# treangenlab/Seqwin

Measured on AMD Instinct MI355X. Metric: Gbp/s minimizer-indexed, higher is better.
Workload: dtype u64

## Files before the change

seqwin_amd/csrc/radix.hip:

```cpp
#include <algorithm>
#include <cstdlib>
#include <cstring>
#include <vector>
#include <map>
#include <mutex>

#include "device.hpp"

namespace sw {
namespace {

constexpr int RS_ITEMS = 16;
#ifdef SW_RS_STAMPS
__device__ unsigned long long *g_rs_stamps = nullptr;
#define RS_STAMP(i)                                                                                        \
    do {                                                                                                   \
        if (g_rs_stamps && (tile & 63u) == 0 && threadIdx.x == 0) g_rs_stamps[(size_t)(tile >> 6) * 16 + (i)] = clock64(); \
    } while (0)
#else
#define RS_STAMP(i) do { } while (0)
#endif
#ifndef RS_LOOK
#define RS_LOOK 4
#endif
// ... 954 lines not shown
        if (!slot) slot = new StateBuf;
        b = slot;
    }
    StateUse u(*b, std::unique_lock<std::mutex>(b->mu));
    if (b->words < words) {
        if (b->p) (void)hipFree(b->p);
        b->p = nullptr;
        b->words = 0;
        const size_t want = words + words / 4;
        SW_HIP(hipMalloc(&b->p, want * 8));
        b->words = want;
        b->epoch = 0;
        SW_HIP(hipMemsetAsync(b->p, 0, want * 8, stream));
    }
    return u;
}
uint32_t next_epoch(StateBuf &b, hipStream_t stream)
{
    if (++b.epoch >= 0xFFFFu) {
        SW_HIP(hipMemsetAsync(b.p, 0, b.words * 8, stream));
        b.epoch = 1;
    }
    return b.epoch;
}

template <int THREADS, int BITS>
void sort_passes(uint64_t *&keys, uint64_t *&alt, uint64_t n, unsigned begin_bit, unsigned end_bit, hipStream_t stream, uint32_t *d_fail,
                 bool perm_hi32, unsigned long long *d_hist_given)
{
    constexpr uint32_t RADIX = 1u << BITS, TILE = THREADS * RS_ITEMS;
    const unsigned n_passes = (end_bit - begin_bit + BITS - 1) / BITS;
    const uint64_t n_tiles = (n + TILE - 1) / TILE;
    const char *kind = SW_AB_GETENV("SEQWIN_AMD_RADIX_KERNEL");
    const bool persistent = !(kind && !strcmp(kind, "classic"));
    uint32_t dbg = 0;
#ifdef SW_RADIX_ABLATION
    if (const char *e = getenv("SEQWIN_AMD_RADIX_DEBUG")) dbg = (uint32_t)atoi(e) & 15u;
#endif
    if (fault_rank()) dbg |= 16u;
    int grid_p = 0;
    if (persistent) {
        static std::mutex &mu = *new std::mutex;
        static std::map<int, int> &grids = *new std::map<int, int>;
        int dev = 0;
        SW_HIP(hipGetDevice(&dev));
        std::lock_guard<std::mutex> lock(mu);
        int &g = grids[dev];
        if (!g) {
            int per_cu = 0;
            hipDeviceProp_t prop;
            SW_HIP(hipGetDeviceProperties(&prop, dev));
            SW_HIP(hipOccupancyMaxActiveBlocksPerMultiprocessor(&per_cu, k_rs_pass_p<THREADS, BITS, 0>, THREADS, 0));
            g = std::max(1, per_cu) * std::max(1, prop.multiProcessorCount);
        }
        grid_p = g;
    }
    const bool atomic_rank = persistent && rank_mode() == 1;
    DevArray<unsigned long long> hist_own(d_hist_given ? 0 : (size_t)n_passes * RADIX), state(persistent ? 0 : (size_t)n_tiles * RADIX);
    std::unique_ptr<StateUse> su(persistent ? new StateUse(state_buf(stream, (size_t)n_tiles * RADIX)) : nullptr);
    StateBuf *sb = su ? &su->b : nullptr;
    struct { unsigned long long *p; } hist{d_hist_given ? d_hist_given : hist_own.p};
    const bool unstable = perm_hi32 && persistent && !SW_AB_GETENV("SEQWIN_AMD_RADIX_STABLE_UNSORT");
    DevArray<unsigned long long> cursor(unstable ? (size_t)RADIX * RS_CURSOR_STRIDE : 0);
    DevArray<uint32_t> tickets(n_passes);
    SW_HIP(hipMemsetAsync(tickets.p, 0, tickets.bytes(), stream));
    if (d_hist_given) {
    } else if (perm_hi32 && begin_bit >= 32) {
        hipLaunchKernelGGL(k_rs_perm_hist<BITS>, dim3(n_passes), dim3(RADIX), 0, stream, n, begin_bit, end_bit, hist.p);
    } else {
        SW_HIP(hipMemsetAsync(hist.p, 0, hist_own.bytes(), stream));
        hipLaunchKernelGGL(k_rs_hist<BITS>, dim3((unsigned)((n + 32767) / 32768)), dim3(256), 0, stream, keys, n, begin_bit, end_bit,
                           n_passes, hist.p);
    }
    SW_HIP(hipGetLastError());
#ifdef SW_RS_STAMPS
    DevArray<unsigned long long> stamps;
    const size_t n_st = (size_t)(n_tiles / 64 + 1) * 16;
    if (getenv("SEQWIN_AMD_STAMPS") && persistent) stamps.alloc(n_st);
#endif
    for (unsigned p = 0; p < n_passes; ++p) {
        const unsigned sh = begin_bit + BITS * p, bits = std::min<unsigned>(BITS, end_bit - sh);
#ifdef SW_RS_STAMPS
        if (stamps.p) {
            SW_HIP(hipMemsetAsync(stamps.p, 0, stamps.bytes(), stream));
            unsigned long long *ptr = stamps.p;
            SW_HIP(hipMemcpyToSymbolAsync(HIP_SYMBOL(g_rs_stamps), &ptr, sizeof ptr, 0, hipMemcpyHostToDevice, stream));
        }
#endif
        unsigned long long *cur = unstable && p == 0 ? cursor.p : nullptr;
        hipLaunchKernelGGL(k_rs_scan<BITS>, dim3(1), dim3(RADIX), 0, stream, hist.p + (size_t)p * RADIX, cur);
        if (!cur && !persistent) SW_HIP(hipMemsetAsync(state.p, 0, state.bytes(), stream));
        if (persistent) {
            const uint32_t epoch = cur ? 0u : next_epoch(*sb, stream);
            auto launch = [&](auto kern) {
                hipLaunchKernelGGL(kern, dim3((unsigned)std::min<uint64_t>(n_tiles, (uint64_t)grid_p)), dim3(THREADS), 0, stream, keys, alt, n,
                                   (uint32_t)n_tiles, sh, bits, hist.p + (size_t)p * RADIX, sb->p, tickets.p + p, d_fail, dbg, cur,
                                   RS_CURSOR_STRIDE, 64u, epoch);
            };
            if (cur ? !ballot_forced() : atomic_rank) launch(k_rs_pass_p<THREADS, BITS, 1>);
            else launch(k_rs_pass_p<THREADS, BITS, 0>);
        } else {
#ifdef SW_AB
            hipLaunchKernelGGL((k_rs_pass<THREADS, BITS>), dim3((unsigned)n_tiles), dim3(THREADS), 0, stream, keys, alt, n, sh, bits,
                               hist.p + (size_t)p * RADIX, state.p, d_fail);
#endif
        }
        SW_HIP(hipGetLastError());
#ifdef SW_RS_STAMPS
        if (stamps.p) {
            std::vector<unsigned long long> hs(n_st);
            SW_HIP(hipStreamSynchronize(stream));
            SW_HIP(hipMemcpy(hs.data(), stamps.p, stamps.bytes(), hipMemcpyDeviceToHost));
            double acc[8] = {0}, look[3] = {0};
            size_t cnt = 0;
            for (size_t t = 0; t + 16 <= n_st; t += 16) {
                if (!hs[t] || !hs[t + 7]) continue;
                for (int i = 1; i <= 7; ++i) acc[i] += (double)(hs[t + i] - hs[t + i - 1]);
                for (int i = 0; i < 3; ++i) look[i] += (double)hs[t + 8 + i];
                ++cnt;
            }
            static const char *nm[] = {"", "rank", "barrier", "totals+scan", "barrier+scatter", "lookback(d0)", "barrier", "write-out"};
            fprintf(stderr, "[rs stamps] %d x %d bits, pass %u, %zu tiles sampled; mean clocks:", THREADS, BITS, p, cnt);
            double sum = 0;
            for (int i = 1; i <= 7; ++i) { fprintf(stderr, " %s=%.0f", nm[i], cnt ? acc[i] / cnt : 0.0); sum += cnt ? acc[i] / cnt : 0.0; }
            fprintf(stderr, " | tile %.0f | look-back of digit 0: %.1f steps, %.1f polls of an unpublished record, %.1f records behind\n", sum,
                    cnt ? look[0] / cnt : 0.0, cnt ? look[1] / cnt : 0.0, cnt ? look[2] / cnt : 0.0);
        }
#endif
        std::swap(keys, alt);
    }
}

}

namespace {
__global__ void k_rs_perm_cursors(unsigned long long *__restrict__ cursor, uint32_t n_groups, uint32_t radix, uint32_t stride,
                                  unsigned group_bits, unsigned digit_shift)
{
    const uint32_t i = blockIdx.x * blockDim.x + threadIdx.x;
    if (i >= n_groups * radix) return;
    const uint64_t g = i / radix, d = i % radix;
    cursor[(size_t)i * stride] = (group_bits < 64 ? g << group_bits : 0ull) + (d << digit_shift);
}
}

bool radix_unsort_perm(uint64_t *&keys, uint64_t *&alt, uint64_t n, unsigned low_bits, unsigned nbit, hipStream_t stream, uint32_t *d_fail)
{
    constexpr int THREADS = 512, BITS = 8;
    constexpr uint32_t RADIX = 1u << BITS, TILE = THREADS * RS_ITEMS;
    if (n == 0 || nbit <= low_bits + 8 || nbit > low_bits + 16 || SW_AB_GETENV("SEQWIN_AMD_RADIX_STABLE_UNSORT")) return false;
    if ((1ull << (low_bits + 8)) % TILE) return false;
    const char *kind = SW_AB_GETENV("SEQWIN_AMD_RADIX_KERNEL");
    if (kind && !strcmp(kind, "classic")) return false;
    const unsigned hi_bits = nbit - low_bits - 8;
    const uint32_t n_groups = (uint32_t)((n + (1ull << (low_bits + 8)) - 1) >> (low_bits + 8));
    const uint64_t n_tiles = (n + TILE - 1) / TILE;
    int dev = 0, per_cu = 0;
    SW_HIP(hipGetDevice(&dev));
    hipDeviceProp_t prop;
    SW_HIP(hipGetDeviceProperties(&prop, dev));
    SW_HIP(hipOccupancyMaxActiveBlocksPerMultiprocessor(&per_cu, k_rs_pass_p<THREADS, BITS, 0>, THREADS, 0));
    const unsigned grid = (unsigned)std::min<uint64_t>(n_tiles, (uint64_t)std::max(1, per_cu) * std::max(1, prop.multiProcessorCount));
    DevArray<unsigned long long> cur_a((size_t)RADIX * RS_CURSOR_STRIDE), cur_b((size_t)n_groups * RADIX);
    DevArray<uint32_t> tickets(2);
    SW_HIP(hipMemsetAsync(tickets.p, 0, 8, stream));
    hipLaunchKernelGGL(k_rs_perm_cursors, dim3(1), dim3(RADIX), 0, stream, cur_a.p, 1u, RADIX, RS_CURSOR_STRIDE, 64u, low_bits + 8);
    hipLaunchKernelGGL(k_rs_perm_cursors, dim3((n_groups * RADIX + 255) / 256), dim3(256), 0, stream, cur_b.p, n_groups, RADIX, 1u,
                       low_bits + 8, low_bits);
    auto pass = ballot_forced() ? k_rs_pass_p<THREADS, BITS, 0> : k_rs_pass_p<THREADS, BITS, 1>;
    hipLaunchKernelGGL(pass, dim3(grid), dim3(THREADS), 0, stream, (const uint64_t *)keys, alt, n, (uint32_t)n_tiles,
                       32u + low_bits + 8, hi_bits, (const unsigned long long *)nullptr, (unsigned long long *)nullptr, tickets.p, d_fail,
                       0u, cur_a.p, RS_CURSOR_STRIDE, 64u, 0u);
    std::swap(keys, alt);
    hipLaunchKernelGGL(pass, dim3(grid), dim3(THREADS), 0, stream, (const uint64_t *)keys, alt, n, (uint32_t)n_tiles, 32u + low_bits,
                       8u, (const unsigned long long *)nullptr, (unsigned long long *)nullptr, tickets.p + 1, d_fail, 0u, cur_b.p, 1u,
                       low_bits + 8, 0u);
    std::swap(keys, alt);
    SW_HIP(hipGetLastError());
    return true;
}

bool radix_pairs_available() { return rank_mode() == 1; }
int radix_rank_mode() { return rank_mode(); }

uint64_t radix_trim_state()
{
    uint64_t freed = 0;
    if (g_state_uses) return 0;
    std::lock_guard<std::mutex> lock(state_registry_mu());
    for (auto &kv : state_registry()) {
        StateBuf &b = *kv.second;
        std::unique_lock<std::mutex> use(b.mu, std::try_to_lock);
        if (!use.owns_lock() || !b.p) continue;
        int cur = -1;
        (void)hipGetDevice(&cur);
        if (cur != kv.first.first) (void)hipSetDevice(kv.first.first);
        (void)hipFree(b.p);
        if (cur != kv.first.first && cur >= 0) (void)hipSetDevice(cur);
        freed += b.words * 8;
        b.p = nullptr;
        b.words = 0;
        b.epoch = 0;
    }
    return freed;
}

void radix_demote_rank()
{
    int dev = 0;
    SW_HIP(hipGetDevice(&dev));
    std::lock_guard<std::mutex> lock(rank_mu());
    rank_modes()[dev] = 0;
}

void radix_sort_pairs32(uint32_t *&keys, uint32_t *&keys_alt, OccPay *&vals, OccPay *&vals_alt, uint64_t n, unsigned end_bit,
                        hipStream_t stream, uint32_t *d_fail, const StageSource *src, const std::function<void()> &after_first,
                        uint32_t *low_out)
{
    constexpr uint32_t RADIX = 1u << RP_BITS, TILE = RP_THREADS * RP_ITEMS;
    if (n == 0 || end_bit == 0) return;
    if (end_bit > 32 || end_bit % RP_BITS) raise(SW_ERR_RUNTIME, "radix_sort_pairs32: key bits must be a multiple of 8 up to 32");
    if (n >= 0xFFFFFFFFull) raise(SW_ERR_RUNTIME, "radix_sort_pairs32: more than 2^32-2 elements");
    const unsigned n_passes = end_bit / RP_BITS;
    const uint64_t n_tiles = (n + TILE - 1) / TILE;
    int grid_p = 0;
    {
        static std::mutex &mu = *new std::mutex;
        static std::map<int, int> &grids = *new std::map<int, int>;
        int dev = 0;
        SW_HIP(hipGetDevice(&dev));
        std::lock_guard<std::mutex> lock(mu);
        int &g = grids[dev];
        if (!g) {
            int per_cu = 0;
            hipDeviceProp_t prop;
            SW_HIP(hipGetDeviceProperties(&prop, dev));
            SW_HIP(hipOccupancyMaxActiveBlocksPerMultiprocessor(&per_cu, k_rs_pair_pass<0>, RP_THREADS, 0));
            g = std::max(1, per_cu) * std::max(1, prop.multiProcessorCount);
        }
        grid_p = g;
    }
    DevArray<unsigned long long> hist((size_t)n_passes * RADIX);
    DevArray<uint32_t> tickets(n_passes);
    SW_HIP(hipMemsetAsync(tickets.p, 0, tickets.bytes(), stream));
    SW_HIP(hipMemsetAsync(hist.p, 0, hist.bytes(), stream));
    StageSource stage{};
    DevArray<uint32_t> chunk_tile;
    DevArray<unsigned long long> chunk_dir;
    if (src && src->rows) {
        stage = *src;
        hipLaunchKernelGGL(k_rs_hist32_rows, dim3((unsigned)((n + 16383) / 16384)), dim3(256), 0, stream,
                           reinterpret_cast<const uint4 *>(src->rows), n, n_passes, hist.p);
    } else if (src) {
        constexpr uint64_t CHUNK = 64 * RP_ITEMS;
        static_assert(TILE == (RP_THREADS / 64) * CHUNK, "a tile is one chunk per wave");
        const uint64_t n_chunks = (n + CHUNK - 1) / CHUNK;
        stage = *src;
        chunk_tile.alloc(n_chunks);
        chunk_dir.alloc(n_chunks * STAGE_ROW);
        stage.chunk_dir = chunk_dir.p;
        hipLaunchKernelGGL(k_rs_chunk_tiles, dim3((stage.n_tiles + 255u) / 256u), dim3(256), 0, stream, stage.tile_count, stage.dst_off,
                           stage.n_tiles, chunk_tile.p);
        hipLaunchKernelGGL(k_rs_stage_prepare, dim3((unsigned)std::min<uint64_t>(2048, (n_chunks + 3) / 4)), dim3(256), 0, stream, stage,
                           (const uint32_t *)chunk_tile.p, n, n_passes, chunk_dir.p, hist.p);
    } else {
        hipLaunchKernelGGL(k_rs_hist32, dim3((unsigned)((n + 65535) / 65536)), dim3(256), 0, stream, keys, n, n_passes, hist.p);
    }
    SW_HIP(hipGetLastError());
    StateUse su = state_buf(stream, (size_t)n_tiles * RADIX);
    StateBuf &sb = su.b;
    const StageSource none{};
    const uint32_t fault = fault_rank();
    for (unsigned p = 0; p < n_passes; ++p) {
        hipLaunchKernelGGL(k_rs_scan<RP_BITS>, dim3(1), dim3(RADIX), 0, stream, hist.p + (size_t)p * RADIX, (unsigned long long *)nullptr);
        const uint32_t epoch = next_epoch(sb, stream);
        const dim3 grid((unsigned)std::min<uint64_t>(n_tiles, (uint64_t)grid_p));
        if (p == 0 && src) {
            auto first = src->rows ? k_rs_pair_pass<2> : k_rs_pair_pass<1>;
            hipLaunchKernelGGL(first, grid, dim3(RP_THREADS), 0, stream, (const uint32_t *)nullptr, (const uint4 *)nullptr,
                               keys_alt, reinterpret_cast<uint4 *>(vals_alt), n, (uint32_t)n_tiles, 0u,
                               (const unsigned long long *)hist.p, sb.p, epoch, tickets.p, d_fail, stage,
                               n_passes == 1 ? low_out : (uint32_t *)nullptr, fault);
            SW_HIP(hipGetLastError());
            if (after_first) after_first();
        } else {
            hipLaunchKernelGGL(k_rs_pair_pass<0>, grid, dim3(RP_THREADS), 0, stream, (const uint32_t *)keys,
                               reinterpret_cast<const uint4 *>(vals), keys_alt, reinterpret_cast<uint4 *>(vals_alt), n, (uint32_t)n_tiles,
                               RP_BITS * p, (const unsigned long long *)(hist.p + (size_t)p * RADIX), sb.p, epoch, tickets.p + p, d_fail,
                               none, p + 1 == n_passes ? low_out : (uint32_t *)nullptr, fault);
            SW_HIP(hipGetLastError());
        }
        std::swap(keys, keys_alt);
        std::swap(vals, vals_alt);
    }
}

namespace {
constexpr uint32_t EB_RADIX = 512, EB_TABLE = EB_RADIX * EB_RADIX, EB_THREADS = 512;
constexpr uint64_t EB_EMPTY = ~0ull;
static_assert(EB_THREADS == EB_RADIX, "k_eb_finish: one bin per thread");
enum : uint32_t { EB_F_OVERFLOW = 1u, EB_F_RANGE = 2u, EB_F_ORDER = 4u };
struct EbInfo {
    unsigned long long n_sentinels;
    uint32_t n_tiles2, max_bucket, flags, n_runs;
};

__global__ __launch_bounds__(EB_RADIX) void k_eb_level1(const unsigned long long *__restrict__ h1, uint32_t tile_keys,
                                                        unsigned long long *__restrict__ cursor, unsigned long long *__restrict__ segtab,
                                                        EbInfo *__restrict__ info)
{
    __shared__ unsigned long long s[EB_RADIX];
    __shared__ uint32_t st[EB_RADIX];
    const uint32_t d = threadIdx.x;
    const unsigned long long c = h1[d];
    const uint32_t tiles = (uint32_t)((c + tile_keys - 1) / tile_keys);
    s[d] = c;
    st[d] = tiles;
    __syncthreads();
    for (uint32_t o = 1; o < EB_RADIX; o <<= 1) {
        const unsigned long long a = d >= o ? s[d - o] : 0;
        const uint32_t b = d >= o ? st[d - o] : 0;
        __syncthreads();
        s[d] += a;
        st[d] += b;
        __syncthreads();
    }
    const unsigned long long first = s[d] - c;
    cursor[(size_t)d * RS_CURSOR_STRIDE] = first;
    uint32_t w = st[d] - tiles;
    for (uint32_t t = 0; t < tiles; ++t)
        segtab[w + t] = seg_pack(first + (uint64_t)t * tile_keys, d, (uint32_t)min((unsigned long long)tile_keys, c - (uint64_t)t * tile_keys));
    if (d == EB_RADIX - 1) info->n_tiles2 = st[d];
}

__global__ __launch_bounds__(1024) void k_eb_count(const uint64_t *__restrict__ in, const unsigned long long *__restrict__ segtab,
                                                   const EbInfo *__restrict__ info, unsigned shift, uint32_t dmask, uint64_t sentinel,
                                                   uint32_t *__restrict__ table, EbInfo *__restrict__ out)
{
    __shared__ uint32_t hist[EB_RADIX];
    __shared__ uint32_t s_sent;
    const uint32_t n_tiles = info->n_tiles2;
    for (uint32_t w = blockIdx.x; w < n_tiles; w += gridDim.x) {
        const unsigned long long seg = segtab[w];
        const uint64_t first = seg_first(seg);
        const uint32_t cnt = seg_count(seg);
        if (threadIdx.x < EB_RADIX) hist[threadIdx.x] = 0;
        if (threadIdx.x == 0) s_sent = 0;
        __syncthreads();
        uint64_t key[RS_ITEMS];
#pragma unroll
        for (int i = 0; i < RS_ITEMS; ++i) {
            const uint32_t li = i * 1024 + threadIdx.x;
            key[i] = li < cnt ? in[first + li] : EB_EMPTY;
        }
        uint32_t sent = 0;
#pragma unroll
        for (int i = 0; i < RS_ITEMS; ++i) {
            if (key[i] == EB_EMPTY) continue;
            if (key[i] == sentinel) ++sent;
            atomicAdd(&hist[(uint32_t)(key[i] >> shift) & dmask], 1u);
        }
        if (sent) atomicAdd(&s_sent, sent);
        __syncthreads();
        if (threadIdx.x < EB_RADIX && hist[threadIdx.x]) atomicAdd(&table[seg_bucket(seg) * EB_RADIX + threadIdx.x], hist[threadIdx.x]);
        if (threadIdx.x == 0 && s_sent) atomicAdd(&out->n_sentinels, (unsigned long long)s_sent);
        __syncthreads();
    }
}

__global__ __launch_bounds__(1024) void k_eb_scan(const uint32_t *__restrict__ cnt, const unsigned long long *__restrict__ n_sent,
                                                  uint32_t sent_at, uint32_t *__restrict__ start, unsigned long long *__restrict__ cursor,
                                                  uint32_t *__restrict__ max_out, uint32_t *__restrict__ total_out)
{
    constexpr uint32_t PER4 = EB_TABLE / 1024 / 4;
    __shared__ uint32_t ws[16], wm[16];
    const uint32_t tid = threadIdx.x, lane = tid & 63u, wave = tid >> 6;
    const uint32_t sent = n_sent ? (uint32_t)*n_sent : 0u;
    const uint4 *cnt4 = reinterpret_cast<const uint4 *>(cnt) + (size_t)tid * PER4;
    uint32_t sum = 0, mx = 0;
#pragma unroll 16
    for (uint32_t j = 0; j < PER4; ++j) {
        const uint4 c = cnt4[j];
        mx = max(max(max(mx, c.x), max(c.y, c.z)), c.w);
        sum += c.x + c.y + c.z + c.w;
    }
    if (n_sent && sent_at / (4 * PER4) == tid) {
        mx = 0;
        for (uint32_t j = 0; j < 4 * PER4; ++j) {
            const uint32_t i = tid * 4 * PER4 + j, c = cnt[i];
            mx = max(mx, c - (i == sent_at ? min(c, sent) : 0u));
        }
    }
    uint32_t incl = sum;
    for (uint32_t o = 1; o < 64; o <<= 1) {
        const uint32_t up = __shfl_up(incl, o, 64);
        if (lane >= o) incl += up;
        mx = max(mx, __shfl_xor(mx, o, 64));
    }
    if (lane == 63) ws[wave] = incl;
    if (lane == 0) wm[wave] = mx;
    __syncthreads();
    uint32_t run = incl - sum;
    for (uint32_t w = 0; w < wave; ++w) run += ws[w];
    uint4 *start4 = reinterpret_cast<uint4 *>(start) + (size_t)tid * PER4;
    ulonglong2 *cur2 = reinterpret_cast<ulonglong2 *>(cursor) + (size_t)tid * PER4 * 2;
#pragma unroll 16
    for (uint32_t j = 0; j < PER4; ++j) {
        const uint4 c = cnt4[j];
        const uint4 st = make_uint4(run, run + c.x, run + c.x + c.y, run + c.x + c.y + c.z);
        start4[j] = st;
        if (cursor) {
            cur2[2 * j] = make_ulonglong2(st.x, st.y);
            cur2[2 * j + 1] = make_ulonglong2(st.z, st.w);
        }
        run = st.w + c.w;
    }
    if (tid == 1023) {
        start[EB_TABLE] = run;
        if (total_out) *total_out = run;
        uint32_t m = 0;
        for (uint32_t w = 0; w < 16; ++w) m = max(m, wm[w]);
        if (max_out) *max_out = m;
    }
}

__global__ __launch_bounds__(EB_THREADS) void k_eb_finish(const uint64_t *__restrict__ in, const uint32_t *__restrict__ start, uint32_t slots,
                                                          unsigned shift1, unsigned shift2, uint32_t mask2, unsigned bin_shift,
                                                          uint32_t bin_mask, uint64_t sentinel,
                                                          uint64_t *__restrict__ tk, uint32_t *__restrict__ tc,
                                                          uint32_t *__restrict__ n_distinct, uint32_t *__restrict__ flags)
{
    extern __shared__ __align__(16) unsigned char eb_lds[];
    unsigned long long *hk = reinterpret_cast<unsigned long long *>(eb_lds);
    uint32_t *hc = reinterpret_cast<uint32_t *>(hk + slots);
    uint16_t *idx = reinterpret_cast<uint16_t *>(hc + slots);
    __shared__ uint32_t bd[EB_RADIX + 1], bk[EB_RADIX], bcur[EB_RADIX], wsd[EB_THREADS / 64], wsk[EB_THREADS / 64];
    __shared__ uint32_t s_over;
    const uint32_t b = EB_TABLE - 1u - blockIdx.x, tid = threadIdx.x, lane = tid & 63u, wave = tid >> 6;
    const uint32_t first = start[b], cnt = start[b + 1] - first;
    if (cnt == 0) return;
    const uint32_t mask = slots - 1u;
    for (uint32_t s = tid; s < slots; s += EB_THREADS) {
        hk[s] = EB_EMPTY;
        hc[s] = 0;
    }
    bd[tid] = 0;
    bk[tid] = 0;
    if (tid == 0) s_over = 0;
    __syncthreads();
    uint32_t bad = 0;
    for (uint32_t j0 = 0; j0 < cnt; j0 += 4 * EB_THREADS) {
        if (*(volatile uint32_t *)&s_over) break;
        uint64_t key[4];
#pragma unroll
        for (int i = 0; i < 4; ++i) {
            const uint32_t j = j0 + i * EB_THREADS + tid;
            key[i] = j < cnt ? in[(uint64_t)first + j] : sentinel;
        }
#pragma unroll
        for (int i = 0; i < 4; ++i) {
            uint64_t k = key[i];
            bool live = k != sentinel;
            if (live && ((uint32_t)(k >> shift1) * EB_RADIX + ((uint32_t)(k >> shift2) & mask2)) != b) {
                bad = 1;
                live = false;
            }
            uint32_t copies = 1;
            const uint64_t any = __ballot(live);
            if (any) {
                const int src = __ffsll((long long)any) - 1;
                const uint64_t k0 = (uint64_t)__shfl((unsigned long long)k, src, 64);
                const uint64_t same = __ballot(live && k == k0);
                if (live && k == k0) {
                    copies = (uint32_t)__popcll(same);
                    live = (int)lane == src;
                }
            }
            if (!live) continue;
            uint32_t h = (uint32_t)((k * 0x9E3779B97F4A7C15ull) >> 40) & mask, probes = 0;
            for (; probes < slots; ++probes) {
                const unsigned long long old = atomicCAS(&hk[h], EB_EMPTY, (unsigned long long)k);
                if (old == EB_EMPTY || old == k) {
                    atomicAdd(&hc[h], copies);
                    break;
                }
                h = (h + 1u) & mask;
            }
            if (probes == slots) s_over = 1;
        }
    }
    if (bad) atomicOr(flags, EB_F_RANGE);
    __syncthreads();
    if (s_over) {
        if (tid == 0) atomicOr(flags, EB_F_OVERFLOW);
        return;
    }
    for (uint32_t s = tid; s < slots; s += EB_THREADS) {
        const uint64_t k = hk[s];
        if (k == EB_EMPTY) continue;
        const uint32_t bin = (uint32_t)(k >> bin_shift) & bin_mask;
        atomicAdd(&bd[bin], 1u);
        atomicAdd(&bk[bin], hc[s]);
    }
    __syncthreads();
    {
        const uint32_t d = bd[tid], c = bk[tid];
        uint32_t id = d, ic = c;
        for (uint32_t o = 1; o < 64; o <<= 1) {
            const uint32_t ud = __shfl_up(id, o, 64), uc = __shfl_up(ic, o, 64);
            if (lane >= o) {
                id += ud;
                ic += uc;
            }
        }
        if (lane == 63) {
            wsd[wave] = id;
            wsk[wave] = ic;
        }
        __syncthreads();
        uint32_t pd = id - d, pc = ic - c;
        for (uint32_t w = 0; w < wave; ++w) {
            pd += wsd[w];
            pc += wsk[w];
        }
        bd[tid] = pd;
        bcur[tid] = pd;
        bk[tid] = pc;
        if (tid == EB_THREADS - 1) bd[EB_RADIX] = pd + d;
    }
    __syncthreads();
    for (uint32_t s = tid; s < slots; s += EB_THREADS) {
        const uint64_t k = hk[s];
        if (k == EB_EMPTY) continue;
        idx[atomicAdd(&bcur[(uint32_t)(k >> bin_shift) & bin_mask], 1u)] = (uint16_t)s;
    }
    __syncthreads();
    const uint32_t n_dist = bd[EB_RADIX];
    if (tid == 0) n_distinct[b] = n_dist;
    for (uint32_t j = tid; j < n_dist; j += EB_THREADS) {
        const uint32_t s = idx[j];
        const uint64_t k = hk[s];
        const uint32_t bin = (uint32_t)(k >> bin_shift) & bin_mask, lo = bd[bin], hi = bd[bin + 1];
        uint32_t less = 0, copies_less = 0;
        for (uint32_t i = lo; i < hi; ++i) {
            const uint32_t s2 = idx[i];
            if (hk[s2] < k) {
                ++less;
                copies_less += hc[s2];
            }
        }
        tk[(uint64_t)first + lo + less] = k;
        tc[(uint64_t)first + lo + less] = first + bk[bin] + copies_less;
    }
}

__global__ __launch_bounds__(256) void k_eb_compact(const uint64_t *__restrict__ tk, const uint32_t *__restrict__ tc,
                                                    const uint32_t *__restrict__ start, const uint32_t *__restrict__ dstart,
                                                    const unsigned long long *__restrict__ n_sentinels, uint64_t *__restrict__ ukeys,
                                                    uint32_t *__restrict__ ucnt, uint32_t *__restrict__ flags)
{
    const uint32_t b = blockIdx.x, d0 = dstart[b], n = dstart[b + 1] - d0;
    if (b == EB_TABLE - 1u && threadIdx.x == 0) ucnt[dstart[EB_TABLE]] = start[EB_TABLE] - (uint32_t)*n_sentinels;
    if (n == 0) return;
    const uint64_t first = start[b];
    uint32_t bad = 0;
    for (uint32_t j = threadIdx.x; j < n; j += 256) {
        const uint64_t k = tk[first + j];
        const uint32_t c = tc[first + j];
        if (j + 1 < n && (tk[first + j + 1] <= k || tc[first + j + 1] <= c)) bad = 1;
        if (c < first || c >= start[b + 1]) bad = 1;
        ukeys[d0 + j] = k;
        ucnt[d0 + j] = c;
    }
    if (bad) atomicOr(flags, EB_F_ORDER);
}
}

int radix_edge_buckets(uint64_t *&keys, uint64_t *&alt, uint64_t m, unsigned key_bits, uint64_t sentinel,
                       const unsigned long long *d_hist_top, uint32_t cap, uint32_t slots, uint64_t *ukeys, uint32_t *ucnt,
                       uint32_t *n_runs, hipStream_t stream, uint32_t *d_fail, bool debug)
{
    constexpr int THREADS = 1024, BITS = 9;
    constexpr uint32_t TILE = THREADS * RS_ITEMS;
    unsigned digit_bits = 0, n_passes = 0;
    radix_layout(key_bits, &digit_bits, &n_passes);
    if (n_passes < 2 || m >= (1ull << 32) - 1 || slots < 64 || slots > 8192 || (slots & (slots - 1))) return 1;
    const unsigned shift1 = (n_passes - 1) * digit_bits, bits1 = key_bits - shift1;
    const unsigned bits2 = std::min<unsigned>(BITS, shift1), shift2 = shift1 - bits2;
    const unsigned bin_bits = std::min<unsigned>(BITS, shift2), bin_shift = shift2 - bin_bits;
    const uint64_t n_tiles = (m + TILE - 1) / TILE, max_tiles2 = n_tiles + EB_RADIX;
    int dev = 0, per_cu = 0;
    SW_HIP(hipGetDevice(&dev));
    hipDeviceProp_t prop;
    SW_HIP(hipGetDeviceProperties(&prop, dev));
    SW_HIP(hipOccupancyMaxActiveBlocksPerMultiprocessor(&per_cu, k_rs_pass_p<THREADS, BITS, 0>, THREADS, 0));
    const unsigned cus = (unsigned)std::max(1, prop.multiProcessorCount);
    const unsigned grid = (unsigned)std::min<uint64_t>(n_tiles, (uint64_t)std::max(1, per_cu) * cus);

    DevArray<unsigned long long> h1(EB_RADIX), cur1((size_t)EB_RADIX * RS_CURSOR_STRIDE), cur2(EB_TABLE), segtab(max_tiles2);
    DevArray<uint32_t> table(EB_TABLE), start(EB_TABLE + 1), tickets(2), flags(1);
    DevArray<EbInfo> info(1);
    SW_HIP(hipMemsetAsync(h1.p, 0, h1.bytes(), stream));
    SW_HIP(hipMemsetAsync(table.p, 0, table.bytes(), stream));
    SW_HIP(hipMemsetAsync(tickets.p, 0, 8, stream));
    SW_HIP(hipMemsetAsync(flags.p, 0, 4, stream));
    SW_HIP(hipMemsetAsync(info.p, 0, sizeof(EbInfo), stream));
    if (d_hist_top)
        SW_HIP(hipMemcpyAsync(h1.p, d_hist_top, (size_t)8 << digit_bits, hipMemcpyDeviceToDevice, stream));
    else
        hipLaunchKernelGGL(k_rs_hist<BITS>, dim3((unsigned)((m + 32767) / 32768)), dim3(256), 0, stream, (const uint64_t *)keys, m, shift1,
                           key_bits, 1u, h1.p);
    hipLaunchKernelGGL(k_eb_level1, dim3(1), dim3(EB_RADIX), 0, stream, (const unsigned long long *)h1.p, TILE, cur1.p, segtab.p, info.p);
    auto pass1 = ballot_forced() ? k_rs_pass_p<THREADS, BITS, 0> : k_rs_pass_p<THREADS, BITS, 1>;
    hipLaunchKernelGGL(pass1, dim3(grid), dim3(THREADS), 0, stream, (const uint64_t *)keys, alt, m, (uint32_t)n_tiles, shift1, bits1,
                       (const unsigned long long *)nullptr, (unsigned long long *)nullptr, tickets.p, d_fail, 0u, cur1.p, RS_CURSOR_STRIDE,
                       64u, 0u);
    std::swap(keys, alt);
    hipLaunchKernelGGL(k_eb_count, dim3((unsigned)std::min<uint64_t>(max_tiles2, (uint64_t)8 * cus)), dim3(1024), 0, stream,
                       (const uint64_t *)keys, (const unsigned long long *)segtab.p, (const EbInfo *)info.p, shift2, (1u << bits2) - 1u,
                       sentinel, table.p, info.p);
    const uint32_t sent_at = (uint32_t)(sentinel >> shift1) * EB_RADIX + ((uint32_t)(sentinel >> shift2) & ((1u << bits2) - 1u));
    hipLaunchKernelGGL(k_eb_scan, dim3(1), dim3(1024), 0, stream, (const uint32_t *)table.p, (const unsigned long long *)&info.p->n_sentinels,
                       sent_at, start.p, cur2.p, &info.p->max_bucket, (uint32_t *)nullptr);
    SW_HIP(hipGetLastError());
    EbInfo hi;
    SW_HIP(hipMemcpyAsync(&hi, info.p, sizeof hi, hipMemcpyDeviceToHost, stream));
    SW_HIP(hipStreamSynchronize(stream));
    if (debug)
        fprintf(stderr, "[edge buckets] %llu keys, %llu sentinels, digits %u+%u+%u of %u bits, largest sub-bucket %u (capacity %u, %u slots)%s\n",
                (unsigned long long)m, hi.n_sentinels, bits1, bits2, bin_bits, key_bits, hi.max_bucket, cap, slots,
                hi.max_bucket > cap ? ": radix passes instead" : "");
    if (hi.max_bucket > cap) return 1;
    auto pass2 = ballot_forced() ? k_rs_pass_p<THREADS, BITS, 0, true> : k_rs_pass_p<THREADS, BITS, 1, true>;
    hipLaunchKernelGGL(pass2, dim3(std::max(1u, std::min(hi.n_tiles2, (uint32_t)(std::max(1, per_cu) * cus)))), dim3(THREADS), 0, stream,
                       (const uint64_t *)keys, alt, m, hi.n_tiles2, shift2, bits2, (const unsigned long long *)segtab.p,
                       (unsigned long long *)nullptr, tickets.p + 1, d_fail, 0u, cur2.p, 1u, 64u, 0u);
    std::swap(keys, alt);
    DevArray<uint32_t> tc(m), n_distinct(EB_TABLE), dstart(EB_TABLE + 1);
    SW_HIP(hipMemsetAsync(n_distinct.p, 0, n_distinct.bytes(), stream));
    uint64_t *tk = alt;
    const size_t lds = (size_t)slots * 14;
    static std::mutex &mu = *new std::mutex;
    {
        std::lock_guard<std::mutex> lock(mu);
        SW_HIP(hipFuncSetAttribute(reinterpret_cast<const void *>(k_eb_finish), hipFuncAttributeMaxDynamicSharedMemorySize, (int)lds));
    }
    hipLaunchKernelGGL(k_eb_finish, dim3(EB_TABLE), dim3(EB_THREADS), lds, stream, (const uint64_t *)keys, (const uint32_t *)start.p, slots,
                       shift1, shift2, (1u << bits2) - 1u, bin_shift, (1u << bin_bits) - 1u, sentinel, tk, tc.p, n_distinct.p, flags.p);
    hipLaunchKernelGGL(k_eb_scan, dim3(1), dim3(1024), 0, stream, (const uint32_t *)n_distinct.p, (const unsigned long long *)nullptr, 0u,
                       dstart.p, (unsigned long long *)nullptr, (uint32_t *)nullptr, &info.p->n_runs);
    hipLaunchKernelGGL(k_eb_compact, dim3(EB_TABLE), dim3(256), 0, stream, (const uint64_t *)tk, (const uint32_t *)tc.p,
                       (const uint32_t *)start.p, (const uint32_t *)dstart.p, (const unsigned long long *)&info.p->n_sentinels, ukeys, ucnt,
                       flags.p);
    SW_HIP(hipGetLastError());
    uint32_t hf = 0;
    SW_HIP(hipMemcpyAsync(&hi, info.p, sizeof hi, hipMemcpyDeviceToHost, stream));
    SW_HIP(hipMemcpyAsync(&hf, flags.p, 4, hipMemcpyDeviceToHost, stream));
    SW_HIP(hipStreamSynchronize(stream));
    if (hf & (EB_F_RANGE | EB_F_ORDER))
        raise(SW_ERR_RUNTIME, "internal error: the edge buckets are out of order (%s)", hf & EB_F_RANGE ? "a key outside its bucket" : "run starts descend");
    if (hf & EB_F_OVERFLOW) {
        if (debug) fprintf(stderr, "[edge buckets] a sub-bucket holds more than %u distinct keys: radix passes instead\n", slots);
        return 1;
    }
    *n_runs = hi.n_runs;
    return 0;
}

static int pick_shape(unsigned bits)
{
    const char *e = SW_TEST_GETENV("SEQWIN_AMD_RADIX_BITS");
    const bool nine = e ? atoi(e) == 9 : (bits + 8) / 9 < (bits + 7) / 8;
    const char *shape = SW_AB_GETENV("SEQWIN_AMD_RADIX_SHAPE");
    if (shape && !strcmp(shape, "1024x8")) return 2;
    if (shape && !strcmp(shape, "512x9")) return 3;
    if (shape && !strcmp(shape, "256x8")) return 4;
    return nine ? 1 : 0;
}

void radix_layout(unsigned bits, unsigned *digit_bits, unsigned *n_passes)
{
    const int sh = pick_shape(bits);
    *digit_bits = (sh == 1 || sh == 3) ? 9u : 8u;
    *n_passes = (bits + *digit_bits - 1) / *digit_bits;
}

void radix_sort_keys64(uint64_t *&keys, uint64_t *&alt, uint64_t n, unsigned begin_bit, unsigned end_bit, hipStream_t stream,
                       uint32_t *d_fail, bool perm_hi32, unsigned long long *d_hist_given, unsigned layout_bits)
{
    if (n == 0 || end_bit <= begin_bit) return;
    if (end_bit - begin_bit > 64) raise(SW_ERR_RUNTIME, "radix_sort_keys64: more than 64 key bits");
    switch (pick_shape(layout_bits ? layout_bits : end_bit - begin_bit)) {
#ifdef SW_AB
    case 2: sort_passes<1024, 8>(keys, alt, n, begin_bit, end_bit, stream, d_fail, perm_hi32, d_hist_given); break;
    case 3: sort_passes<512, 9>(keys, alt, n, begin_bit, end_bit, stream, d_fail, perm_hi32, d_hist_given); break;
    case 4: sort_passes<256, 8>(keys, alt, n, begin_bit, end_bit, stream, d_fail, perm_hi32, d_hist_given); break;
#endif
    case 1: sort_passes<1024, 9>(keys, alt, n, begin_bit, end_bit, stream, d_fail, perm_hi32, d_hist_given); break;
    default: sort_passes<512, 8>(keys, alt, n, begin_bit, end_bit, stream, d_fail, perm_hi32, d_hist_given); break;
    }
}

}
```

Measured before the change: 473.1.

## Pack edge-bucket hash counts into keys, launch only live sub-buckets, batch probes

The scan kernel now builds a compact list of non-empty sub-buckets, ordered largest index first, so the finish and compact kernels launch one workgroup per live bucket instead of all 262144. The finish kernel gains a packed mode that stores the low key bits and the count in one 64-bit LDS word, which cuts LDS per slot from 14 to 10 bytes and removes the separate count atomic. It also prefetches the next key batch, runs hash probes for four keys in an interleaved loop, and unrolls the rank loop. The packed mode falls back to radix passes when the bits do not fit, and it adds complexity and optional timing stamps.

```diff
diff --git a/seqwin_amd/csrc/radix.hip b/seqwin_amd/csrc/radix.hip
--- a/seqwin_amd/csrc/radix.hip
+++ b/seqwin_amd/csrc/radix.hip
@@ -1280,7 +1280,7 @@
 enum : uint32_t { EB_F_OVERFLOW = 1u, EB_F_RANGE = 2u, EB_F_ORDER = 4u };
 struct EbInfo {
     unsigned long long n_sentinels;
-    uint32_t n_tiles2, max_bucket, flags, n_runs;
+    uint32_t n_tiles2, max_bucket, flags, n_runs, n_live, pad;
 };
 
 __global__ __launch_bounds__(EB_RADIX) void k_eb_level1(const unsigned long long *__restrict__ h1, uint32_t tile_keys,
@@ -1348,19 +1348,21 @@
 
 __global__ __launch_bounds__(1024) void k_eb_scan(const uint32_t *__restrict__ cnt, const unsigned long long *__restrict__ n_sent,
                                                   uint32_t sent_at, uint32_t *__restrict__ start, unsigned long long *__restrict__ cursor,
-                                                  uint32_t *__restrict__ max_out, uint32_t *__restrict__ total_out)
+                                                  uint32_t *__restrict__ max_out, uint32_t *__restrict__ total_out,
+                                                  uint4 *__restrict__ live, uint32_t *__restrict__ n_live_out)
 {
     constexpr uint32_t PER4 = EB_TABLE / 1024 / 4;
-    __shared__ uint32_t ws[16], wm[16];
+    __shared__ uint32_t ws[16], wm[16], wz[16];
     const uint32_t tid = threadIdx.x, lane = tid & 63u, wave = tid >> 6;
     const uint32_t sent = n_sent ? (uint32_t)*n_sent : 0u;
     const uint4 *cnt4 = reinterpret_cast<const uint4 *>(cnt) + (size_t)tid * PER4;
-    uint32_t sum = 0, mx = 0;
+    uint32_t sum = 0, mx = 0, nz = 0;
 #pragma unroll 16
     for (uint32_t j = 0; j < PER4; ++j) {
         const uint4 c = cnt4[j];
         mx = max(max(max(mx, c.x), max(c.y, c.z)), c.w);
         sum += c.x + c.y + c.z + c.w;
+        nz += (c.x != 0) + (c.y != 0) + (c.z != 0) + (c.w != 0);
     }
     if (n_sent && sent_at / (4 * PER4) == tid) {
         mx = 0;
@@ -1369,17 +1371,30 @@
             mx = max(mx, c - (i == sent_at ? min(c, sent) : 0u));
         }
     }
-    uint32_t incl = sum;
+    uint32_t incl = sum, inz = nz;
     for (uint32_t o = 1; o < 64; o <<= 1) {
-        const uint32_t up = __shfl_up(incl, o, 64);
-        if (lane >= o) incl += up;
+        const uint32_t up = __shfl_up(incl, o, 64), uz = __shfl_up(inz, o, 64);
+        if (lane >= o) {
+            incl += up;
+            inz += uz;
+        }
         mx = max(mx, __shfl_xor(mx, o, 64));
     }
-    if (lane == 63) ws[wave] = incl;
+    if (lane == 63) {
+        ws[wave] = incl;
+        wz[wave] = inz;
+    }
     if (lane == 0) wm[wave] = mx;
     __syncthreads();
-    uint32_t run = incl - sum;
-    for (uint32_t w = 0; w < wave; ++w) run += ws[w];
+    uint32_t run = incl - sum, below = inz - nz, n_live = 0;
+    for (uint32_t w = 0; w < 16; ++w) {
+        if (w < wave) {
+            run += ws[w];
+            below += wz[w];
+        }
+        n_live += wz[w];
+    }
+    uint32_t at = n_live - 1u - below;
     uint4 *start4 = reinterpret_cast<uint4 *>(start) + (size_t)tid * PER4;
     ulonglong2 *cur2 = reinterpret_cast<ulonglong2 *>(cursor) + (size_t)tid * PER4 * 2;
 #pragma unroll 16
@@ -1391,96 +1406,162 @@
             cur2[2 * j] = make_ulonglong2(st.x, st.y);
             cur2[2 * j + 1] = make_ulonglong2(st.z, st.w);
         }
+        if (live) {
+            const uint32_t id = (tid * PER4 + j) * 4;
+            if (c.x) live[at--] = make_uint4(id, st.x, c.x, 0u);
+            if (c.y) live[at--] = make_uint4(id + 1, st.y, c.y, 0u);
+            if (c.z) live[at--] = make_uint4(id + 2, st.z, c.z, 0u);
+            if (c.w) live[at--] = make_uint4(id + 3, st.w, c.w, 0u);
+        }
         run = st.w + c.w;
     }
     if (tid == 1023) {
         start[EB_TABLE] = run;
         if (total_out) *total_out = run;
+        if (n_live_out) *n_live_out = n_live;
         uint32_t m = 0;
         for (uint32_t w = 0; w < 16; ++w) m = max(m, wm[w]);
         if (max_out) *max_out = m;
     }
 }
 
-__global__ __launch_bounds__(EB_THREADS) void k_eb_finish(const uint64_t *__restrict__ in, const uint32_t *__restrict__ start, uint32_t slots,
+#ifdef SW_RS_STAMPS
+__device__ unsigned long long *g_eb_stamps = nullptr;
+constexpr uint32_t EB_ST_EVERY = 16, EB_ST_WORDS = 16;
+#define EB_STAMP(i) do { if (st) st[i] = clock64(); } while (0)
+#define EB_STAMP_ADD(i, since) do { if (st) { const unsigned long long t_ = clock64(); st[i] += t_ - (since); (since) = t_; } } while (0)
+#else
+#define EB_STAMP(i) do { } while (0)
+#define EB_STAMP_ADD(i, since) do { } while (0)
+#endif
+
+template <bool PACKED>
+__global__ __launch_bounds__(EB_THREADS) void k_eb_finish(const uint64_t *__restrict__ in, const uint4 *__restrict__ live, uint32_t slots,
                                                           unsigned shift1, unsigned shift2, uint32_t mask2, unsigned bin_shift,
-                                                          uint32_t bin_mask, uint64_t sentinel,
+                                                          uint32_t bin_mask, unsigned cb, uint64_t sentinel,
                                                           uint64_t *__restrict__ tk, uint32_t *__restrict__ tc,
                                                           uint32_t *__restrict__ n_distinct, uint32_t *__restrict__ flags)
 {
     extern __shared__ __align__(16) unsigned char eb_lds[];
     unsigned long long *hk = reinterpret_cast<unsigned long long *>(eb_lds);
     uint32_t *hc = reinterpret_cast<uint32_t *>(hk + slots);
-    uint16_t *idx = reinterpret_cast<uint16_t *>(hc + slots);
+    uint16_t *idx = PACKED ? reinterpret_cast<uint16_t *>(hk + slots) : reinterpret_cast<uint16_t *>(hc + slots);
     __shared__ uint32_t bd[EB_RADIX + 1], bk[EB_RADIX], bcur[EB_RADIX], wsd[EB_THREADS / 64], wsk[EB_THREADS / 64];
     __shared__ uint32_t s_over;
-    const uint32_t b = EB_TABLE - 1u - blockIdx.x, tid = threadIdx.x, lane = tid & 63u, wave = tid >> 6;
-    const uint32_t first = start[b], cnt = start[b + 1] - first;
-    if (cnt == 0) return;
+    const uint32_t tid = threadIdx.x, lane = tid & 63u, wave = tid >> 6;
+#ifdef SW_RS_STAMPS
+    unsigned long long *st = g_eb_stamps && tid == 0 && blockIdx.x % EB_ST_EVERY == 0 ? g_eb_stamps + (size_t)(blockIdx.x / EB_ST_EVERY) * EB_ST_WORDS : nullptr;
+    unsigned long long st_t = 0;
+#endif
+    EB_STAMP(0);
+    const uint4 me = live[blockIdx.x];
     const uint32_t mask = slots - 1u;
     for (uint32_t s = tid; s < slots; s += EB_THREADS) {
         hk[s] = EB_EMPTY;
-        hc[s] = 0;
+        if (!PACKED) hc[s] = 0;
     }
     bd[tid] = 0;
     bk[tid] = 0;
     if (tid == 0) s_over = 0;
-    __syncthreads();
+    const uint32_t b = me.x, first = me.y, cnt = me.z;
+    const uint64_t low_mask = (1ull << shift2) - 1ull, count_mask = (1ull << cb) - 1ull;
+    const uint64_t high = ((uint64_t)(b / EB_RADIX) << shift1) | ((uint64_t)(b % EB_RADIX) << shift2);
+    uint64_t nxt[4];
+#pragma unroll
+    for (int i = 0; i < 4; ++i) {
+        const uint32_t j = i * EB_THREADS + tid;
+        nxt[i] = j < cnt ? in[(uint64_t)first + j] : sentinel;
+    }
+    EB_STAMP(1);
+    __syncthreads();
+    EB_STAMP(2);
+#ifdef SW_RS_STAMPS
+    if (st) st_t = clock64();
+#endif
     uint32_t bad = 0;
     for (uint32_t j0 = 0; j0 < cnt; j0 += 4 * EB_THREADS) {
         if (*(volatile uint32_t *)&s_over) break;
         uint64_t key[4];
 #pragma unroll
+        for (int i = 0; i < 4; ++i) key[i] = nxt[i];
+        if (j0 + 4 * EB_THREADS < cnt) {
+#pragma unroll
+            for (int i = 0; i < 4; ++i) {
+                const uint32_t j = j0 + 4 * EB_THREADS + i * EB_THREADS + tid;
+                nxt[i] = j < cnt ? in[(uint64_t)first + j] : sentinel;
+            }
+        }
+        uint32_t cp[4], h[4];
+        unsigned long long w[4];
+#pragma unroll
         for (int i = 0; i < 4; ++i) {
-            const uint32_t j = j0 + i * EB_THREADS + tid;
-            key[i] = j < cnt ? in[(uint64_t)first + j] : sentinel;
-        }
-#pragma unroll
-        for (int i = 0; i < 4; ++i) {
-            uint64_t k = key[i];
-            bool live = k != sentinel;
-            if (live && ((uint32_t)(k >> shift1) * EB_RADIX + ((uint32_t)(k >> shift2) & mask2)) != b) {
+            const uint64_t k = key[i];
+            bool alive = k != sentinel;
+            if (alive && ((uint32_t)(k >> shift1) * EB_RADIX + ((uint32_t)(k >> shift2) & mask2)) != b) {
                 bad = 1;
-                live = false;
+                alive = false;
             }
             uint32_t copies = 1;
-            const uint64_t any = __ballot(live);
+            const uint64_t any = __ballot(alive);
             if (any) {
                 const int src = __ffsll((long long)any) - 1;
                 const uint64_t k0 = (uint64_t)__shfl((unsigned long long)k, src, 64);
-                const uint64_t same = __ballot(live && k == k0);
-                if (live && k == k0) {
+                const uint64_t same = __ballot(alive && k == k0);
+                if (alive && k == k0) {
                     copies = (uint32_t)__popcll(same);
-                    live = (int)lane == src;
+                    alive = (int)lane == src;
                 }
             }
-            if (!live) continue;
-            uint32_t h = (uint32_t)((k * 0x9E3779B97F4A7C15ull) >> 40) & mask, probes = 0;
-            for (; probes < slots; ++probes) {
-                const unsigned long long old = atomicCAS(&hk[h], EB_EMPTY, (unsigned long long)k);
-                if (old == EB_EMPTY || old == k) {
-                    atomicAdd(&hc[h], copies);
-                    break;
+            cp[i] = alive ? copies : 0u;
+            h[i] = (uint32_t)((k * 0x9E3779B97F4A7C15ull) >> 40) & mask;
+            w[i] = PACKED ? ((k & low_mask) << cb) | copies : (unsigned long long)k;
+        }
+        EB_STAMP_ADD(3, st_t);
+        for (uint32_t probes = 0; cp[0] | cp[1] | cp[2] | cp[3]; ++probes) {
+            if (probes == slots) {
+                s_over = 1;
+                break;
+            }
+            unsigned long long old[4];
+#pragma unroll
+            for (int i = 0; i < 4; ++i)
+                if (cp[i]) old[i] = atomicCAS(&hk[h[i]], EB_EMPTY, w[i]);
+#pragma unroll
+            for (int i = 0; i < 4; ++i) {
+                if (!cp[i]) continue;
+                if (PACKED) {
+                    if (old[i] == EB_EMPTY) cp[i] = 0;
+                    else if ((old[i] >> cb) == (w[i] >> cb)) {
+                        atomicAdd(&hk[h[i]], (unsigned long long)cp[i]);
+                        cp[i] = 0;
+                    } else h[i] = (h[i] + 1u) & mask;
+                } else {
+                    if (old[i] == EB_EMPTY || old[i] == w[i]) {
+                        atomicAdd(&hc[h[i]], cp[i]);
+                        cp[i] = 0;
+                    } else h[i] = (h[i] + 1u) & mask;
                 }
-                h = (h + 1u) & mask;
-            }
-            if (probes == slots) s_over = 1;
-        }
+            }
+        }
+        EB_STAMP_ADD(4, st_t);
     }
     if (bad) atomicOr(flags, EB_F_RANGE);
     __syncthreads();
+    EB_STAMP(5);
     if (s_over) {
         if (tid == 0) atomicOr(flags, EB_F_OVERFLOW);
         return;
     }
+    const unsigned wbin_shift = PACKED ? bin_shift + cb : bin_shift;
     for (uint32_t s = tid; s < slots; s += EB_THREADS) {
         const uint64_t k = hk[s];
         if (k == EB_EMPTY) continue;
-        const uint32_t bin = (uint32_t)(k >> bin_shift) & bin_mask;
+        const uint32_t bin = (uint32_t)(k >> wbin_shift) & bin_mask;
         atomicAdd(&bd[bin], 1u);
-        atomicAdd(&bk[bin], hc[s]);
-    }
-    __syncthreads();
+        atomicAdd(&bk[bin], PACKED ? (uint32_t)(k & count_mask) : hc[s]);
+    }
+    __syncthreads();
+    EB_STAMP(6);
     {
         const uint32_t d = bd[tid], c = bk[tid];
         uint32_t id = d, ic = c;
@@ -1497,9 +1578,9 @@
         }
         __syncthreads();
         uint32_t pd = id - d, pc = ic - c;
-        for (uint32_t w = 0; w < wave; ++w) {
-            pd += wsd[w];
-            pc += wsk[w];
+        for (uint32_t w2 = 0; w2 < wave; ++w2) {
+            pd += wsd[w2];
+            pc += wsk[w2];
         }
         bd[tid] = pd;
         bcur[tid] = pd;
@@ -1507,46 +1588,71 @@
         if (tid == EB_THREADS - 1) bd[EB_RADIX] = pd + d;
     }
     __syncthreads();
+    EB_STAMP(7);
     for (uint32_t s = tid; s < slots; s += EB_THREADS) {
         const uint64_t k = hk[s];
         if (k == EB_EMPTY) continue;
-        idx[atomicAdd(&bcur[(uint32_t)(k >> bin_shift) & bin_mask], 1u)] = (uint16_t)s;
-    }
-    __syncthreads();
+        idx[atomicAdd(&bcur[(uint32_t)(k >> wbin_shift) & bin_mask], 1u)] = (uint16_t)s;
+    }
+    __syncthreads();
+    EB_STAMP(8);
     const uint32_t n_dist = bd[EB_RADIX];
     if (tid == 0) n_distinct[b] = n_dist;
     for (uint32_t j = tid; j < n_dist; j += EB_THREADS) {
         const uint32_t s = idx[j];
         const uint64_t k = hk[s];
-        const uint32_t bin = (uint32_t)(k >> bin_shift) & bin_mask, lo = bd[bin], hi = bd[bin + 1];
+        const uint32_t bin = (uint32_t)(k >> wbin_shift) & bin_mask, lo = bd[bin], hi = bd[bin + 1];
         uint32_t less = 0, copies_less = 0;
-        for (uint32_t i = lo; i < hi; ++i) {
-            const uint32_t s2 = idx[i];
-            if (hk[s2] < k) {
-                ++less;
-                copies_less += hc[s2];
-            }
-        }
-        tk[(uint64_t)first + lo + less] = k;
+        for (uint32_t i = lo; i < hi; i += 4) {
+            uint32_t s2[4];
+            unsigned long long k2[4];
+            uint32_t c2[4];
+#pragma unroll
+            for (int u = 0; u < 4; ++u) s2[u] = i + u < hi ? idx[i + u] : s;
+#pragma unroll
+            for (int u = 0; u < 4; ++u) {
+                k2[u] = hk[s2[u]];
+                c2[u] = PACKED ? 0u : hc[s2[u]];
+            }
+#pragma unroll
+            for (int u = 0; u < 4; ++u) {
+                if (PACKED ? (k2[u] >> cb) < (k >> cb) : k2[u] < k) {
+                    ++less;
+                    copies_less += PACKED ? (uint32_t)(k2[u] & count_mask) : c2[u];
+                }
+            }
+        }
+        tk[(uint64_t)first + lo + less] = PACKED ? high | (k >> cb) : k;
         tc[(uint64_t)first + lo + less] = first + bk[bin] + copies_less;
     }
+#ifdef SW_RS_STAMPS
+    if (st) {
+        st[9] = clock64();
+        st[10] = cnt;
+        st[11] = n_dist;
+    }
+#endif
 }
 
 __global__ __launch_bounds__(256) void k_eb_compact(const uint64_t *__restrict__ tk, const uint32_t *__restrict__ tc,
-                                                    const uint32_t *__restrict__ start, const uint32_t *__restrict__ dstart,
+                                                    const uint4 *__restrict__ live, uint32_t n_live, const uint32_t *__restrict__ start,
+                                                    const uint32_t *__restrict__ dstart,
                                                     const unsigned long long *__restrict__ n_sentinels, uint64_t *__restrict__ ukeys,
                                                     uint32_t *__restrict__ ucnt, uint32_t *__restrict__ flags)
 {
-    const uint32_t b = blockIdx.x, d0 = dstart[b], n = dstart[b + 1] - d0;
-    if (b == EB_TABLE - 1u && threadIdx.x == 0) ucnt[dstart[EB_TABLE]] = start[EB_TABLE] - (uint32_t)*n_sentinels;
+    if (blockIdx.x == 0 && threadIdx.x == 0) ucnt[dstart[EB_TABLE]] = start[EB_TABLE] - (uint32_t)*n_sentinels;
+    if (blockIdx.x >= n_live) return;
+    const uint4 me = live[blockIdx.x];
+    const uint32_t b = me.x, d0 = dstart[b], n = dstart[b + 1] - d0;
     if (n == 0) return;
-    const uint64_t first = start[b];
+    const uint64_t first = me.y;
+    const uint32_t end = me.y + me.z;
     uint32_t bad = 0;
     for (uint32_t j = threadIdx.x; j < n; j += 256) {
         const uint64_t k = tk[first + j];
         const uint32_t c = tc[first + j];
         if (j + 1 < n && (tk[first + j + 1] <= k || tc[first + j + 1] <= c)) bad = 1;
-        if (c < first || c >= start[b + 1]) bad = 1;
+        if (c < first || c >= end) bad = 1;
         ukeys[d0 + j] = k;
         ucnt[d0 + j] = c;
     }
@@ -1577,6 +1683,7 @@
 
     DevArray<unsigned long long> h1(EB_RADIX), cur1((size_t)EB_RADIX * RS_CURSOR_STRIDE), cur2(EB_TABLE), segtab(max_tiles2);
     DevArray<uint32_t> table(EB_TABLE), start(EB_TABLE + 1), tickets(2), flags(1);
+    DevArray<uint4> live(EB_TABLE);
     DevArray<EbInfo> info(1);
     SW_HIP(hipMemsetAsync(h1.p, 0, h1.bytes(), stream));
     SW_HIP(hipMemsetAsync(table.p, 0, table.bytes(), stream));
@@ -1599,16 +1706,36 @@
                        sentinel, table.p, info.p);
     const uint32_t sent_at = (uint32_t)(sentinel >> shift1) * EB_RADIX + ((uint32_t)(sentinel >> shift2) & ((1u << bits2) - 1u));
     hipLaunchKernelGGL(k_eb_scan, dim3(1), dim3(1024), 0, stream, (const uint32_t *)table.p, (const unsigned long long *)&info.p->n_sentinels,
-                       sent_at, start.p, cur2.p, &info.p->max_bucket, (uint32_t *)nullptr);
+                       sent_at, start.p, cur2.p, &info.p->max_bucket, (uint32_t *)nullptr, live.p, &info.p->n_live);
     SW_HIP(hipGetLastError());
     EbInfo hi;
     SW_HIP(hipMemcpyAsync(&hi, info.p, sizeof hi, hipMemcpyDeviceToHost, stream));
     SW_HIP(hipStreamSynchronize(stream));
-    if (debug)
-        fprintf(stderr, "[edge buckets] %llu keys, %llu sentinels, digits %u+%u+%u of %u bits, largest sub-bucket %u (capacity %u, %u slots)%s\n",
+    unsigned cb = 1;
+    while (cb < 32 && (hi.max_bucket >> cb)) ++cb;
+    const bool eligible = shift2 + cb <= 63;
+    bool packed = eligible;
+    if (const char *e = SW_TEST_GETENV("SEQWIN_AMD_EDGE_FINISH")) packed = !strcmp(e, "packed");
+    const bool refused = packed && !eligible;
+    const size_t lds = (size_t)slots * (packed ? 10 : 14);
+    auto finish = packed ? k_eb_finish<true> : k_eb_finish<false>;
+    static std::mutex &mu = *new std::mutex;
+    static int lds_set[2] = {0, 0};
+    {
+        std::lock_guard<std::mutex> lock(mu);
+        lds_set[packed] = std::max(lds_set[packed], (int)lds);
+        SW_HIP(hipFuncSetAttribute(reinterpret_cast<const void *>(finish), hipFuncAttributeMaxDynamicSharedMemorySize, lds_set[packed]));
+    }
+    if (debug) {
+        int resident = 0;
+        SW_HIP(hipOccupancyMaxActiveBlocksPerMultiprocessor(&resident, finish, EB_THREADS, lds));
+        fprintf(stderr, "[edge buckets] %llu keys, %llu sentinels, digits %u+%u+%u of %u bits, largest sub-bucket %u (capacity %u, %u slots)%s; "
+                        "%u live sub-buckets, %s slots%s, %d workgroups per CU\n",
                 (unsigned long long)m, hi.n_sentinels, bits1, bits2, bin_bits, key_bits, hi.max_bucket, cap, slots,
-                hi.max_bucket > cap ? ": radix passes instead" : "");
-    if (hi.max_bucket > cap) return 1;
+                hi.max_bucket > cap ? ": radix passes instead" : "", hi.n_live, packed ? "packed" : "plain",
+                refused ? " do not fit: radix passes instead" : "", resident);
+    }
+    if (hi.max_bucket > cap || refused) return 1;
     auto pass2 = ballot_forced() ? k_rs_pass_p<THREADS, BITS, 0, true> : k_rs_pass_p<THREADS, BITS, 1, true>;
     hipLaunchKernelGGL(pass2, dim3(std::max(1u, std::min(hi.n_tiles2, (uint32_t)(std::max(1, per_cu) * cus)))), dim3(THREADS), 0, stream,
                        (const uint64_t *)keys, alt, m, hi.n_tiles2, shift2, bits2, (const unsigned long long *)segtab.p,
@@ -1617,19 +1744,53 @@
     DevArray<uint32_t> tc(m), n_distinct(EB_TABLE), dstart(EB_TABLE + 1);
     SW_HIP(hipMemsetAsync(n_distinct.p, 0, n_distinct.bytes(), stream));
     uint64_t *tk = alt;
-    const size_t lds = (size_t)slots * 14;
-    static std::mutex &mu = *new std::mutex;
-    {
-        std::lock_guard<std::mutex> lock(mu);
-        SW_HIP(hipFuncSetAttribute(reinterpret_cast<const void *>(k_eb_finish), hipFuncAttributeMaxDynamicSharedMemorySize, (int)lds));
-    }
-    hipLaunchKernelGGL(k_eb_finish, dim3(EB_TABLE), dim3(EB_THREADS), lds, stream, (const uint64_t *)keys, (const uint32_t *)start.p, slots,
-                       shift1, shift2, (1u << bits2) - 1u, bin_shift, (1u << bin_bits) - 1u, sentinel, tk, tc.p, n_distinct.p, flags.p);
+#ifdef SW_RS_STAMPS
+    DevArray<unsigned long long> stamps;
+    const size_t n_st = (size_t)(hi.n_live / EB_ST_EVERY + 1) * EB_ST_WORDS;
+    if (getenv("SEQWIN_AMD_STAMPS")) {
+        stamps.alloc(n_st);
+        SW_HIP(hipMemsetAsync(stamps.p, 0, stamps.bytes(), stream));
+        unsigned long long *ptr = stamps.p;
+        SW_HIP(hipMemcpyToSymbolAsync(HIP_SYMBOL(g_eb_stamps), &ptr, sizeof ptr, 0, hipMemcpyHostToDevice, stream));
+    }
+#endif
+    if (hi.n_live)
+        hipLaunchKernelGGL(finish, dim3(hi.n_live), dim3(EB_THREADS), lds, stream, (const uint64_t *)keys, (const uint4 *)live.p, slots, shift1,
+                           shift2, (1u << bits2) - 1u, bin_shift, (1u << bin_bits) - 1u, cb, sentinel, tk, tc.p, n_distinct.p, flags.p);
+#ifdef SW_RS_STAMPS
+    if (stamps.p) {
+        std::vector<unsigned long long> hs(n_st);
+        SW_HIP(hipStreamSynchronize(stream));
+        SW_HIP(hipMemcpy(hs.data(), stamps.p, stamps.bytes(), hipMemcpyDeviceToHost));
+        unsigned long long *none = nullptr;
+        SW_HIP(hipMemcpyToSymbol(HIP_SYMBOL(g_eb_stamps), &none, sizeof none));
+        double acc[10] = {0}, keys_sum = 0, dist_sum = 0;
+        size_t cnt = 0;
+        for (size_t t = 0; t + EB_ST_WORDS <= n_st; t += EB_ST_WORDS) {
+            if (!hs[t] || !hs[t + 9] || hs[t + 10] <= 2 * 4 * EB_THREADS || hs[t + 10] > 3 * 4 * EB_THREADS) continue;
+            acc[1] += (double)(hs[t + 1] - hs[t]);
+            acc[2] += (double)(hs[t + 2] - hs[t + 1]);
+            acc[3] += (double)hs[t + 3];
+            acc[4] += (double)hs[t + 4];
+            acc[5] += (double)(hs[t + 5] - hs[t + 2]) - (double)hs[t + 3] - (double)hs[t + 4];
+            for (int i = 6; i <= 9; ++i) acc[i] += (double)(hs[t + i] - hs[t + i - 1]);
+            keys_sum += (double)hs[t + 10];
+            dist_sum += (double)hs[t + 11];
+            ++cnt;
+        }
+        static const char *nm[] = {"", "entry+list", "init+barrier", "merge(+key wait)", "probes", "loop barrier", "bin count", "scan", "scatter", "rank+store"};
+        fprintf(stderr, "[eb stamps] %s slots, %zu workgroups of 3 steps sampled (mean %.0f keys, %.0f distinct); mean clocks:", packed ? "packed" : "plain",
+                cnt, cnt ? keys_sum / cnt : 0.0, cnt ? dist_sum / cnt : 0.0);
+        double sum = 0;
+        for (int i = 1; i <= 9; ++i) { fprintf(stderr, " %s=%.0f", nm[i], cnt ? acc[i] / cnt : 0.0); sum += cnt ? acc[i] / cnt : 0.0; }
+        fprintf(stderr, " | workgroup %.0f\n", sum);
+    }
+#endif
     hipLaunchKernelGGL(k_eb_scan, dim3(1), dim3(1024), 0, stream, (const uint32_t *)n_distinct.p, (const unsigned long long *)nullptr, 0u,
-                       dstart.p, (unsigned long long *)nullptr, (uint32_t *)nullptr, &info.p->n_runs);
-    hipLaunchKernelGGL(k_eb_compact, dim3(EB_TABLE), dim3(256), 0, stream, (const uint64_t *)tk, (const uint32_t *)tc.p,
-                       (const uint32_t *)start.p, (const uint32_t *)dstart.p, (const unsigned long long *)&info.p->n_sentinels, ukeys, ucnt,
-                       flags.p);
+                       dstart.p, (unsigned long long *)nullptr, (uint32_t *)nullptr, &info.p->n_runs, (uint4 *)nullptr, (uint32_t *)nullptr);
+    hipLaunchKernelGGL(k_eb_compact, dim3(std::max(1u, hi.n_live)), dim3(256), 0, stream, (const uint64_t *)tk, (const uint32_t *)tc.p,
+                       (const uint4 *)live.p, hi.n_live, (const uint32_t *)start.p, (const uint32_t *)dstart.p,
+                       (const unsigned long long *)&info.p->n_sentinels, ukeys, ucnt, flags.p);
     SW_HIP(hipGetLastError());
     uint32_t hf = 0;
     SW_HIP(hipMemcpyAsync(&hi, info.p, sizeof hi, hipMemcpyDeviceToHost, stream));
```

After: 488.6, median of 6. 3.3% higher.
